# tontinton/dbeel

Measured on NVIDIA H100. Metric: compaction throughput MB/s (input bytes) at 1/2/4/8 H100 vs CPU shards, higher is better.
Workload: dtype u8

## Files before the change

dbeel_b200/csrc/kernels.cuh:

```cuda
#pragma once
#include <cuda_runtime.h>
#include <stdint.h>

#include "device_fns.cuh"

namespace dbeel {


struct RunDesc {
    const uint8_t *data;
    uint64_t data_len;
    uint64_t off_base;
    const uint4 *index;
    uint32_t n_in;
    uint32_t base;
};

struct Seg {
    uint32_t start, len;
};

enum : uint32_t {
    kFlagTruncated = 1u,
    kFlagUnsorted = 2u,
// ... 497 lines not shown
    }
    if (total) atomicAdd(&s_total, total);
    if (trunc) atomicAdd(&s_trunc, trunc);
    if (flags) atomicOr(&s_flags, flags);
    __syncthreads();
    for (uint32_t l = 0; l < p.n_levels; l++) {
        const uint32_t pairs = p.nseg[l + 1];
        uint32_t carry = 0;
        for (uint32_t j0 = 0; j0 < pairs; j0 += 1024) {
            const uint32_t j = j0 + tid;
            uint32_t tiles = 0;
            if (j < pairs) {
                const Seg a = p.seg[l][2 * j];
                const uint32_t blen = (2 * j + 1 < p.nseg[l]) ? p.seg[l][2 * j + 1].len : 0;
                p.seg[l + 1][j].start = a.start;
                p.seg[l + 1][j].len = a.len + blen;
                const uint32_t tl = (p.fin_tile && l + 1 == p.n_levels) ? p.fin_tile : (uint32_t)kMergeTile;
                tiles = (a.len + blen + tl - 1) / tl;
            }
            unsigned long long vb = 0, tb;
            uint32_t vc = tiles, tc;
            __syncthreads();
            block_excl_scan_1024(vb, vc, s_b, s_c, &tb, &tc);
            if (j < pairs) p.tile_base[l][j] = carry + vc;
            carry += tc;
        }
        if (tid == 0) p.tile_base[l][pairs] = carry;
        __syncthreads();
    }
    if (tid == 0) {
        c->total = s_total;
        c->span = p.n_groups ? p.n_total : s_total;
        c->runs_truncated = s_trunc;
        c->flags = c->flags | s_flags;
    }
}


__global__ void k_flush_prefix_init(Params p) {
    pdl_trigger();
    pdl_wait();
    if (threadIdx.x || blockIdx.x) return;
    Ctl *c = p.ctl;
    const uint8_t *ptr;
    uint32_t kl = 0;
    uint32_t L = 0;
    const RunDesc &rd = p.runs[p.flush_ref_run];
    if (rd.n_in && safe_key(rd, 0, &ptr, &kl)) {
        L = kl < kMaxPrefix ? kl : kMaxPrefix;
        for (uint32_t i = 0; i < L; i++) c->prefix[i] = __ldg(ptr + i);
    }
    c->prefix_len = L;
}

__global__ void __launch_bounds__(256) k_flush_prefix(Params p) {
    pdl_trigger();
    pdl_wait();
    Ctl *c = p.ctl;
    uint32_t g = blockIdx.x * 256u + threadIdx.x;
    uint32_t L = c->prefix_len;
    if (g < p.n_total && L) {
        const uint32_t r = find_run(p, g);
        const uint8_t *ptr;
        uint32_t kl;
        if (safe_key(p.runs[r], g - p.runs[r].base, &ptr, &kl)) {
            uint32_t m = kl < L ? kl : L, i = 0;
            while (i < m && __ldg(ptr + i) == c->prefix[i]) i++;
            L = i;
        }
    }
    for (int o = 16; o; o >>= 1) {
        uint32_t other = __shfl_xor_sync(0xFFFFFFFFu, L, o);
        L = other < L ? other : L;
    }
    if ((threadIdx.x & 31) == 0 && L < c->prefix_len) atomicMin(&c->prefix_len, L);
}

__device__ __forceinline__ bool arrival_less(const Params &p, uint32_t skip, const Rec &a, const Rec &b) {
    int und;
    int c = rec_cmp_window(a, b, &und);
    if (und) c = full_key_cmp(p, a.w, b.w, skip);
    return c < 0 || (c == 0 && a.w < b.w);
}

__global__ void __launch_bounds__(kMergeThreads) k_block_sort(Params p) {
    pdl_trigger();
    pdl_wait();
    __shared__ Rec s[kMergeTile + kMergeVT + 1];
    const Seg sg = p.seg[0][blockIdx.x];
    const uint32_t base = sg.start;
    const uint32_t n = sg.len;
    if (n == 0) return;
    const uint32_t tid = threadIdx.x;
    const uint32_t skip = p.ctl->prefix_len + kWindowBytes;
    Rec inf;
    inf.x = inf.y = inf.z = inf.w = 0xFFFFFFFFu;
    for (uint32_t i = tid; i < (uint32_t)kMergeTile; i += kMergeThreads) s[i] = i < n ? ld_rec(&p.rec_a[base + i]) : inf;
    __syncthreads();
    Rec r[kMergeVT];
#pragma unroll
    for (int i = 0; i < kMergeVT; i++) r[i] = s[tid * kMergeVT + i];
#pragma unroll
    for (int pass = 0; pass < kMergeVT; pass++) {
#pragma unroll
        for (int i = pass & 1; i + 1 < kMergeVT; i += 2) {
            if (arrival_less(p, skip, r[i + 1], r[i])) { Rec t = r[i]; r[i] = r[i + 1]; r[i + 1] = t; }
        }
    }
    __syncthreads();
#pragma unroll
    for (int i = 0; i < kMergeVT; i++) s[tid * kMergeVT + i] = r[i];
    __syncthreads();
    for (uint32_t len = kMergeVT; len < (uint32_t)kMergeTile; len <<= 1) {
        const uint32_t d0 = tid * kMergeVT;
        const uint32_t pair = d0 / (2 * len);
        const uint32_t diag = d0 - pair * 2 * len;
        const Rec *A = s + pair * 2 * len;
        const Rec *B = A + len;
        uint32_t lo = diag > len ? diag - len : 0;
        uint32_t hi = diag < len ? diag : len;
        while (lo < hi) {
            uint32_t mid = (lo + hi) >> 1;
            if (!arrival_less(p, skip, B[diag - 1 - mid], A[mid])) lo = mid + 1; else hi = mid;
        }
        uint32_t ai = lo, bi = diag - lo;
        Rec ak = A[ai < len ? ai : len - 1], bk = B[bi < len ? bi : len - 1];
#pragma unroll
        for (int i = 0; i < kMergeVT; i++) {
            bool has_a = ai < len, has_b = bi < len;
            bool take_b = has_b && (!has_a || arrival_less(p, skip, bk, ak));
            r[i] = take_b ? bk : ak;
            if (take_b) { bi++; if (bi < len) bk = B[bi]; } else { ai++; if (ai < len) ak = A[ai]; }
        }
        __syncthreads();
#pragma unroll
        for (int i = 0; i < kMergeVT; i++) s[d0 + i] = r[i];
        __syncthreads();
    }
    for (uint32_t i = tid; i < n; i += kMergeThreads) st_rec(&p.rec_a[base + i], s[i]);
}


__device__ __forceinline__ uint32_t find_pair(const uint32_t *tb, uint32_t pairs, uint32_t v, uint32_t slope) {
    uint32_t lo = 0, hi = pairs;
    while (hi - lo > 1) {
        uint32_t mid = (lo + hi) >> 1;
        if (tb[mid] + slope * mid <= v) lo = mid; else hi = mid;
    }
    return lo;
}

constexpr int kPartitionThreads = 256;

__global__ void __launch_bounds__(kPartitionThreads) k_merge_partition(Params p, uint32_t level, const Rec *src) {
    pdl_trigger();
    pdl_wait();
    const uint32_t pairs = p.nseg[level + 1];
    const uint32_t *tb = p.tile_base[level];
    const uint32_t n_bound = tb[pairs] + pairs;
    const uint32_t idx = (blockIdx.x * (uint32_t)kPartitionThreads + threadIdx.x) >> 5, lane = threadIdx.x & 31;
    if (idx >= n_bound) return;
    const uint32_t skip = p.ctl->prefix_len + kWindowBytes;
    uint32_t j = find_pair(tb, pairs, idx, 1);
    uint32_t t = idx - (tb[j] + j);
    Seg a = p.seg[level][2 * j];
    Seg b;
    b.start = 0; b.len = 0;
    if (2 * j + 1 < p.nseg[level]) b = p.seg[level][2 * j + 1];
    const bool fin = p.fin_tile && level + 1 == p.n_levels;
    uint64_t d64 = (uint64_t)t * (fin ? p.fin_tile : (uint32_t)kMergeTile);
    uint32_t n = a.len + b.len;
    uint32_t diag = d64 < n ? (uint32_t)d64 : n;
    uint32_t lo = diag > b.len ? diag - b.len : 0;
    uint32_t hi = diag < a.len ? diag : a.len;
    while (lo < hi) {
        const uint32_t range = hi - lo;
        const uint32_t step = range >= 32 ? range >> 5 : 1;
        const uint32_t mid = lo + lane * step + (step - 1);
        bool pr = false;
        if (mid < hi) {
            Rec ra = ld_rec(&src[a.start + mid]);
            Rec rb = ld_rec(&src[b.start + (diag - 1 - mid)]);
            pr = !key_less(p, skip, rb, ra);
        }
        const uint32_t cnt = __popc(__ballot_sync(0xFFFFFFFFu, pr));
        const uint32_t first_false = lo + cnt * step + (step - 1);
        lo = lo + cnt * step;
        if (cnt < 32 && first_false < hi) hi = first_false;
        else if (range < 32) hi = lo;
    }
    if (lane == 0) {
        p.part[idx] = lo;
        if (!fin) p.bnd[idx] = make_uint4(a.start + lo, b.start + (diag - lo), a.start + diag, j);
        if (t * (uint64_t)(fin ? p.fin_tile : (uint32_t)kMergeTile) < n) p.tile_bnd[tb[j] + t] = idx;
    }
    if (fin) {
        uint32_t ext = 0;
        if (diag > 0 && diag < n) {
            const uint32_t ai = lo, bi = diag - lo;
            Rec K;
            if (ai == 0) K = ld_rec(&src[b.start + bi - 1]);
            else if (bi == 0) K = ld_rec(&src[a.start + ai - 1]);
            else {
                const Rec ka = ld_rec(&src[a.start + ai - 1]), kb = ld_rec(&src[b.start + bi - 1]);
                K = key_less(p, skip, ka, kb) ? kb : ka;
            }
            const bool ea = ai + lane < a.len && key_equal(p, skip, K, ld_rec(&src[a.start + ai + lane]));
            const bool eb = bi + lane < b.len && key_equal(p, skip, K, ld_rec(&src[b.start + bi + lane]));
            const uint32_t ma = __ballot_sync(0xFFFFFFFFu, ea), mb = __ballot_sync(0xFFFFFFFFu, eb);
            uint32_t xa = (uint32_t)__ffs((int)~ma), xb = (uint32_t)__ffs((int)~mb);
            xa = xa ? xa - 1 : 32;
            xb = xb ? xb - 1 : 32;
            ext = (xa > 31 ? 31u : xa) | ((xb > 31 ? 31u : xb) << 8);
        }
        if (lane == 0) {
            p.part_ext[idx] = ext;
            p.bnd[idx] = make_uint4(a.start + lo + (ext & 0xFF), b.start + (diag - lo) + (ext >> 8), a.start + diag, j);
        }
    }
}

__global__ void __launch_bounds__(kMergeThreads, 4) k_merge(Params p, uint32_t level, const Rec *src, Rec *dst) {
    pdl_trigger();
    pdl_wait();
    __shared__ Rec s[kMergeTile + kMergeVT + 1];
    const uint32_t pairs = p.nseg[level + 1];
    const uint32_t *tb = p.tile_base[level];
    const uint32_t tile = blockIdx.x;
    if (tile >= tb[pairs]) return;
    const uint32_t tid = threadIdx.x;
    const uint32_t skip = p.ctl->prefix_len + kWindowBytes;
    uint32_t j = find_pair(tb, pairs, tile, 0);
    uint32_t t = tile - tb[j];
    Seg a = p.seg[level][2 * j];
    Seg b;
    b.start = 0; b.len = 0;
    if (2 * j + 1 < p.nseg[level]) b = p.seg[level][2 * j + 1];
    const uint32_t pidx = tb[j] + j + t;
    const uint32_t a0 = p.part[pidx], a1 = p.part[pidx + 1];
    const uint32_t total = a.len + b.len;
    const uint32_t diag0 = t * kMergeTile;
    const uint32_t diag1 = diag0 + kMergeTile < total ? diag0 + kMergeTile : total;
    const uint32_t b0 = diag0 - a0, b1 = diag1 - a1;
    const uint32_t nA = a1 - a0, nB = b1 - b0, n = nA + nB;

    for (uint32_t i = tid; i < nA; i += kMergeThreads) s[i] = ld_rec(&src[a.start + a0 + i]);
    for (uint32_t i = tid; i < nB; i += kMergeThreads) s[nA + i] = ld_rec(&src[b.start + b0 + i]);
    __syncthreads();

    uint32_t d = tid * kMergeVT;
    if (d > n) d = n;
    uint32_t lo = d > nB ? d - nB : 0;
    uint32_t hi = d < nA ? d : nA;
    while (lo < hi) {
        uint32_t mid = (lo + hi) >> 1;
        if (!key_less_smem(p, skip, &s[nA + d - 1 - mid], &s[mid])) lo = mid + 1; else hi = mid;
    }
    uint32_t ai = lo, bi = d - lo;
    Rec ak = s[ai], bk = s[nA + bi];
    Rec out[kMergeVT];
#pragma unroll
    for (int i = 0; i < kMergeVT; i++) {
        bool has_a = ai < nA, has_b = bi < nB;
        bool take_b = has_b && (!has_a || key_less(p, skip, bk, ak));
        out[i] = take_b ? bk : ak;
        if (take_b) { bi++; bk = s[nA + bi]; } else { ai++; ak = s[ai]; }
    }
    Rec *o = dst + a.start + diag0;
    __syncthreads();
#pragma unroll
    for (int i = 0; i < kMergeVT; i++)
        if (d + i < n) s[d + i] = out[i];
    __syncthreads();
    for (uint32_t i = tid; i < n; i += kMergeThreads) st_rec(&o[i], s[i]);
}


struct MergeDesc {
    uint32_t a_src, n_a, b_src, n_b, dst;
};

__device__ __forceinline__ MergeDesc merge_desc(const Params &p, uint32_t level, uint32_t tile) {
    const uint32_t pairs = p.nseg[level + 1];
    const uint32_t *tb = p.tile_base[level];
    MergeDesc d;
    d.a_src = d.n_a = d.b_src = d.n_b = d.dst = 0;
    if (tile >= tb[pairs]) return d;
    const uint32_t j = find_pair(tb, pairs, tile, 0);
    const uint32_t t = tile - tb[j];
    const Seg a = p.seg[level][2 * j];
    Seg b;
    b.start = 0; b.len = 0;
    if (2 * j + 1 < p.nseg[level]) b = p.seg[level][2 * j + 1];
    const uint32_t pidx = tb[j] + j + t;
    const uint32_t a0 = p.part[pidx], a1 = p.part[pidx + 1];
    const uint32_t total = a.len + b.len;
    const uint32_t diag0 = t * kMergeTile;
    const uint32_t diag1 = diag0 + kMergeTile < total ? diag0 + kMergeTile : total;
    d.a_src = a.start + a0;
    d.n_a = a1 - a0;
    d.b_src = b.start + (diag0 - a0);
    d.n_b = (diag1 - a1) - (diag0 - a0);
    d.dst = a.start + diag0;
    return d;
}

constexpr int kMergeBufRecs = kMergeTile + kMergeVT + 1;


__device__ __forceinline__ uint32_t smem_u32(const void *p) { return (uint32_t)__cvta_generic_to_shared(p); }
__device__ __forceinline__ void mbar_init(uint64_t *bar, uint32_t count) {
    asm volatile("mbarrier.init.shared::cta.b64 [%0], %1;" ::"r"(smem_u32(bar)), "r"(count) : "memory");
}
__device__ __forceinline__ void mbar_expect_tx(uint64_t *bar, uint32_t bytes) {
    asm volatile("mbarrier.arrive.expect_tx.shared::cta.b64 _, [%0], %1;" ::"r"(smem_u32(bar)), "r"(bytes) : "memory");
}
__device__ __forceinline__ bool mbar_try_wait(uint64_t *bar, uint32_t parity) {
    uint32_t ok;
    asm volatile("{\n .reg .pred p;\n mbarrier.try_wait.parity.shared::cta.b64 p, [%1], %2;\n selp.u32 %0, 1, 0, p;\n}"
                 : "=r"(ok) : "r"(smem_u32(bar)), "r"(parity) : "memory");
    return ok != 0;
}
__device__ __forceinline__ void tma_load_1d(void *smem_dst, const void *gmem_src, uint32_t bytes, uint64_t *bar) {
    asm volatile("cp.async.bulk.shared::cluster.global.mbarrier::complete_tx::bytes [%0], [%1], %2, [%3];" ::"r"(smem_u32(smem_dst)),
                 "l"(gmem_src), "r"(bytes), "r"(smem_u32(bar)) : "memory");
}
__device__ __forceinline__ void tma_store_1d(void *gmem_dst, const void *smem_src, uint32_t bytes) {
    asm volatile("cp.async.bulk.global.shared::cta.bulk_group [%0], [%1], %2;" ::"l"(gmem_dst), "r"(smem_u32(smem_src)), "r"(bytes) : "memory");
}

__global__ void __launch_bounds__(kMergeThreads, kMergeCtasPerSM) k_merge_tma(Params p, uint32_t level, const Rec *src, Rec *dst) {
    pdl_trigger();
    pdl_wait();
    extern __shared__ __align__(128) uint8_t s_raw[];
    Rec *bufs[2] = {reinterpret_cast<Rec *>(s_raw), reinterpret_cast<Rec *>(s_raw) + kMergeBufRecs};
    __shared__ __align__(8) uint64_t s_bar[2];
    const uint32_t tid = threadIdx.x;
    const uint32_t skip = p.ctl->prefix_len + kWindowBytes;
    const uint32_t n_tiles = p.tile_base[level][p.nseg[level + 1]];
    const uint32_t G = gridDim.x;
    uint32_t tile = blockIdx.x;
    if (tile >= n_tiles) return;
    if (tid == 0) {
        mbar_init(&s_bar[0], 1);
        mbar_init(&s_bar[1], 1);
        asm volatile("fence.mbarrier_init.release.cluster;" ::: "memory");
    }
    __syncthreads();

    auto issue = [&](const MergeDesc &d, Rec *buf, uint64_t *bar) {
        mbar_expect_tx(bar, (d.n_a + d.n_b) * 16u);
        if (d.n_a) tma_load_1d(buf, &src[d.a_src], d.n_a * 16u, bar);
        if (d.n_b) tma_load_1d(buf + d.n_a, &src[d.b_src], d.n_b * 16u, bar);
    };

    auto ld_bidx = [&](uint32_t t) -> uint32_t { return t < n_tiles ? __ldg(&p.tile_bnd[t]) : 0xFFFFFFFFu; };
    auto mk_desc = [&](uint32_t bidx) -> MergeDesc {
        MergeDesc d;
        d.a_src = d.n_a = d.b_src = d.n_b = d.dst = 0;
        if (bidx == 0xFFFFFFFFu) return d;
        const uint4 b0 = __ldg(&p.bnd[bidx]), b1 = __ldg(&p.bnd[bidx + 1]);
        d.a_src = b0.x; d.n_a = b1.x - b0.x;
        d.b_src = b0.y; d.n_b = b1.y - b0.y;
        d.dst = b0.z;
        return d;
    };
    MergeDesc cur = mk_desc(ld_bidx(tile));
    MergeDesc nxt = mk_desc(ld_bidx(tile + G));
    uint32_t bidx2 = ld_bidx(tile + 2 * G);
    if (tid == 0) issue(cur, bufs[0], &s_bar[0]);
    for (uint32_t q = 0;; q++) {
        Rec *s = bufs[q & 1];
        const bool has_next = tile + G < n_tiles;
        if (tid == 0 && has_next) {
            asm volatile("cp.async.bulk.wait_group.read 0;" ::: "memory");
            issue(nxt, bufs[(q + 1) & 1], &s_bar[(q + 1) & 1]);
        }
        const MergeDesc nn = mk_desc(bidx2);
        const uint32_t bidx3 = ld_bidx(tile + 3 * G);
        while (!mbar_try_wait(&s_bar[q & 1], (q >> 1) & 1)) {}

        const uint32_t nA = cur.n_a, nB = cur.n_b, n = nA + nB;
        uint32_t d = tid * kMergeVT;
        if (d > n) d = n;
        uint32_t lo = d > nB ? d - nB : 0;
        uint32_t hi = d < nA ? d : nA;
        while (lo < hi) {
            uint32_t mid = (lo + hi) >> 1;
            if (!key_less_smem(p, skip, &s[nA + d - 1 - mid], &s[mid])) lo = mid + 1; else hi = mid;
        }
        uint32_t ai = lo, bi = d - lo;
        Rec ak = s[ai], bk = s[nA + bi];
        Rec out[kMergeVT];
#pragma unroll
        for (int i = 0; i < kMergeVT; i++) {
            bool has_a = ai < nA, has_b = bi < nB;
            bool take_b = has_b && (!has_a || key_less(p, skip, bk, ak));
            out[i] = take_b ? bk : ak;
            if (take_b) { bi++; bk = s[nA + bi]; } else { ai++; ak = s[ai]; }
        }
        __syncthreads();
#pragma unroll
        for (int i = 0; i < kMergeVT; i++)
            if (d + i < n) s[d + i] = out[i];
        asm volatile("fence.proxy.async.shared::cta;" ::: "memory");
        __syncthreads();
        if (tid == 0) {
            tma_store_1d(dst + cur.dst, s, n * 16u);
            asm volatile("cp.async.bulk.commit_group;" ::: "memory");
        }
        if (!has_next) break;
        tile += G;
        cur = nxt;
        nxt = nn;
        bidx2 = bidx3;
    }
    if (tid == 0) asm volatile("cp.async.bulk.wait_group 0;" ::: "memory");
}


__device__ __forceinline__ void ld_ts(const uint8_t *entry, uint32_t full_size, uint64_t *lo, uint64_t *hi) {
    const uint8_t *t = entry + full_size - 16;
    *lo = ld_u64_unaligned(t);
    *hi = ld_u64_unaligned(t + 8);
}

#ifndef DBEEL_RESOLVE_MINB
#define DBEEL_RESOLVE_MINB 14
#endif
constexpr unsigned long long kScanAgg = 1, kScanPrefix = 2;

__device__ __forceinline__ unsigned long long ld_volatile_u64(const unsigned long long *q) {
    unsigned long long v;
    asm volatile("ld.volatile.global.u64 %0, [%1];" : "=l"(v) : "l"(q) : "memory");
    return v;
}
__device__ __forceinline__ void st_volatile_u64(unsigned long long *q, unsigned long long v) {
    asm volatile("st.volatile.global.u64 [%0], %1;" ::"l"(q), "l"(v) : "memory");
}

#ifndef DBEEL_RESOLVE_FUSED_MINB
#define DBEEL_RESOLVE_FUSED_MINB 12
#endif
template <bool kNarrow, bool kFused, bool kHashRec>
__global__ void __launch_bounds__(kResolveThreads, kFused ? DBEEL_RESOLVE_FUSED_MINB : DBEEL_RESOLVE_MINB) k_resolve(Params p, const Rec *m, uint4 *res) {
    pdl_trigger();
    pdl_wait();
    constexpr int NT = kResolveThreads;
    __shared__ Rec s_rec[NT + 2];
    __shared__ unsigned long long s_entry[NT];
    __shared__ uint32_t s_ks[NT], s_fs[NT];
    __shared__ unsigned long long s_tlo[NT], s_thi[NT];
    __shared__ uint8_t s_eqn[NT];
    const Ctl *c = p.ctl;
    const uint32_t tid = threadIdx.x;
    const uint32_t span = c->span;
    __shared__ uint32_t s_tile;
    if (kFused) {
        if (tid == 0) s_tile = atomicAdd(p.scan_ticket, 1u);
        __syncthreads();
    }
    const uint32_t tile_id = kFused ? s_tile : blockIdx.x;
    const uint32_t i0 = tile_id * NT;
    if (i0 >= span) return;
    const uint32_t skip = c->prefix_len + kWindowBytes;
    const uint32_t i = i0 + tid;
    uint32_t lim_lo = 0, lim_hi = c->total;
    int keep_tombstones = p.keep_tombstones;
    if (p.n_groups && i < span) {
        const uint32_t g = find_group(p, i);
        const Seg sl = p.seg[p.n_levels][g];
        lim_lo = sl.start;
        lim_hi = sl.start + sl.len;
        if (p.groups) keep_tombstones = p.groups[g].keep_tombstones;
    }

    for (uint32_t k = tid; k < NT + 2; k += NT) {
        int64_t gi = (int64_t)i0 - 1 + k;
        if (gi >= 0 && gi < (int64_t)span) s_rec[k] = ld_rec(&m[gi]);
    }
    __syncthreads();

    const bool active = i < span && i < lim_hi;
    bool eq_prev = false, eq_next = false;
// ... 1352 lines not shown
```

dbeel_b200/csrc/merge_final.cuh:

```cuda
#pragma once
#include "kernels.cuh"

namespace dbeel {

constexpr int kFinThreads = kMergeThreads;
constexpr int kFinVT = kMergeVT;
constexpr int kFinTile = kMergeTile;
constexpr int kFinNominal = kFinTile - 64;
constexpr int kFinBufRecs = kFinTile + 8;
constexpr int kFinMaxRunsSmem = 64;
#ifndef DBEEL_FIN_CTAS
#define DBEEL_FIN_CTAS 2
#endif
constexpr uint32_t kFinSmem = 2u * kFinBufRecs * 16u + 2u * kFinTile * 8u + (uint32_t)kFinTile + 16u;

struct FinDesc {
    uint32_t a_src, n_a, b_src, n_b;
    uint32_t a_end, b_end;
    uint32_t diag0;
    uint32_t nb;
};

template <bool kNarrow>
__global__ void __launch_bounds__(kFinThreads, DBEEL_FIN_CTAS) k_merge_final(Params p, uint32_t level, const Rec *src) {
    constexpr int NT = kFinThreads, VT = kFinVT;
    extern __shared__ __align__(128) uint8_t f_raw[];
    Rec *bufs[2] = {reinterpret_cast<Rec *>(f_raw), reinterpret_cast<Rec *>(f_raw) + kFinBufRecs};
    unsigned long long *s_tlo = reinterpret_cast<unsigned long long *>(f_raw + 2u * kFinBufRecs * 16u);
    unsigned long long *s_thi = s_tlo + kFinTile;
    uint8_t *s_flag = reinterpret_cast<uint8_t *>(s_thi + kFinTile);
    __shared__ __align__(8) uint64_t s_bar[2];
    __shared__ Rec s_bnd[5];
    __shared__ unsigned long long s_wb[NT / 32];
    __shared__ uint32_t s_wc[NT / 32];
    __shared__ unsigned long long s_pref_b;
    __shared__ uint32_t s_pref_c;
    __shared__ uint32_t s_first[NT / 32];
    __shared__ uint32_t s_rbase[kFinMaxRunsSmem + 1];
    __shared__ uint8_t s_rlut[256];
    __shared__ const uint4 *s_rindex[kFinMaxRunsSmem];
    __shared__ const uint8_t *s_rdata[kFinMaxRunsSmem];

    pdl_trigger();
    pdl_wait();
    const uint32_t tid = threadIdx.x, lane = tid & 31, warp = tid >> 5;
    const uint32_t skip = p.ctl->prefix_len + kWindowBytes;
    const uint32_t n_tiles = p.tile_base[level][p.nseg[level + 1]];
    const uint32_t G = gridDim.x;
    uint32_t tile = blockIdx.x;
    if (tile >= n_tiles) return;
    const bool runs_cached = p.n_runs <= (uint32_t)kFinMaxRunsSmem;
    uint32_t lut_shift = 0;
    while (((uint64_t)p.n_total >> lut_shift) > 256) lut_shift++;
    if (runs_cached) {
        for (uint32_t r = tid; r < p.n_runs; r += NT) {
            s_rbase[r] = p.runs[r].base;
            s_rindex[r] = p.runs[r].index;
            s_rdata[r] = p.runs[r].data;
        }
        if (tid == 0) s_rbase[p.n_runs] = 0xFFFFFFFFu;
        s_rlut[tid] = (uint8_t)find_run(p, (uint32_t)(((uint64_t)tid << lut_shift) < p.n_total ? (uint64_t)tid << lut_shift : p.n_total - 1));
    }
    if (tid == 0) {
        mbar_init(&s_bar[0], 1);
        mbar_init(&s_bar[1], 1);
        asm volatile("fence.mbarrier_init.release.cluster;" ::: "memory");
    }
    __syncthreads();

    auto run_of = [&](uint32_t gid) -> uint32_t {
        if (!runs_cached) return find_run(p, gid);
        uint32_t r = s_rlut[gid >> lut_shift];
        while (s_rbase[r + 1] <= gid) r++;
        return r;
    };
    auto index_ptr = [&](uint32_t gid, uint32_t r) -> const uint4 * {
        return runs_cached ? s_rindex[r] + (gid - s_rbase[r]) : p.runs[r].index + (gid - p.runs[r].base);
    };
    auto data_ptr = [&](uint32_t r) -> const uint8_t * { return runs_cached ? s_rdata[r] : p.runs[r].data; };

    auto issue = [&](const FinDesc &d, Rec *buf, uint64_t *bar) {
        const uint32_t ap = d.nb & 1u, an = (d.nb >> 1) & 1u, bp = (d.nb >> 2) & 1u, bn = (d.nb >> 3) & 1u;
        const uint32_t ca = d.n_a + ap + an, cb = d.n_b + bp + bn;
        asm volatile("fence.proxy.async.shared::cta;" ::: "memory");
        mbar_expect_tx(bar, (ca + cb) * 16u);
        if (ca) tma_load_1d(buf + 1 - ap, &src[d.a_src - ap], ca * 16u, bar);
        if (cb) tma_load_1d(buf + d.n_a + 3 - bp, &src[d.b_src - bp], cb * 16u, bar);
    };

    const Seg segA = p.seg[level][0];
    Seg segB;
    segB.start = 0; segB.len = 0;
    if (p.nseg[level] > 1) segB = p.seg[level][1];
    auto ld_bidx = [&](uint32_t t) -> uint32_t { return t < n_tiles ? __ldg(&p.tile_bnd[t]) : 0xFFFFFFFFu; };
    auto mk_desc = [&](uint32_t bidx) -> FinDesc {
        FinDesc d;
        d.a_src = d.n_a = d.b_src = d.n_b = d.a_end = d.b_end = d.diag0 = d.nb = 0;
        if (bidx == 0xFFFFFFFFu) return d;
        const uint4 b0 = __ldg(&p.bnd[bidx]), b1 = __ldg(&p.bnd[bidx + 1]);
        d.a_src = b0.x; d.n_a = b1.x - b0.x;
        d.b_src = b0.y; d.n_b = b1.y - b0.y;
        d.a_end = segA.start + segA.len;
        d.b_end = segB.start + segB.len;
        d.diag0 = b0.z;
        d.nb = (b0.x > segA.start ? 1u : 0u) | (b1.x < d.a_end ? 2u : 0u) | (b0.y > segB.start ? 4u : 0u) | (b1.y < d.b_end ? 8u : 0u);
        return d;
    };
    FinDesc cur = mk_desc(ld_bidx(tile));
    FinDesc nxt = mk_desc(ld_bidx(tile + G));
    uint32_t bidx2 = ld_bidx(tile + 2 * G);
    if (tid == 0) issue(cur, bufs[0], &s_bar[0]);
    const int keep_tombstones = p.keep_tombstones;

    for (uint32_t q = 0;; q++) {
        Rec *s = bufs[q & 1];
        uint4 *s4 = reinterpret_cast<uint4 *>(s);
        const bool has_next = tile + G < n_tiles;
        if (tid == 0 && has_next) issue(nxt, bufs[(q + 1) & 1], &s_bar[(q + 1) & 1]);
        const FinDesc nn = mk_desc(bidx2);
        const uint32_t bidx3 = ld_bidx(tile + 3 * G);
        while (!mbar_try_wait(&s_bar[q & 1], (q >> 1) & 1)) {}

        const uint32_t nA = cur.n_a, nB = cur.n_b, n = nA + nB;
        const Rec *A = s + 1, *B = s + nA + 3;
        uint32_t d = tid * VT;
        if (d > n) d = n;
        Rec me[VT + 1];
        {
            uint32_t lo = d > nB ? d - nB : 0;
            uint32_t hi = d < nA ? d : nA;
            while (lo < hi) {
                const uint32_t mid = (lo + hi) >> 1;
                if (!key_less_smem(p, skip, &B[d - 1 - mid], &A[mid])) lo = mid + 1; else hi = mid;
            }
            uint32_t ai = lo, bi = d - lo;
            Rec ak = A[ai], bk = B[bi];
#pragma unroll
            for (int i = 0; i < VT; i++) {
                const bool has_a = ai < nA, has_b = bi < nB;
                const bool take_b = has_b && (!has_a || key_less(p, skip, bk, ak));
                me[i] = take_b ? bk : ak;
                if (take_b) { bi++; bk = B[bi]; } else { ai++; ak = A[ai]; }
            }
            if (tid == 0) {
                s_bnd[0] = s[0];
                s_bnd[1] = s[nA + 1];
                s_bnd[2] = s[nA + 2];
                s_bnd[3] = s[nA + 3 + nB];
            }
            __syncthreads();
            if (d < n) s[d] = me[0];
            if (d + VT - 1 < n) s[d + VT - 1] = me[VT - 1];
#pragma unroll
            for (int i = 0; i < VT; i++)
                if (d + i == n - 1) s_bnd[4] = me[i];
        }
        __syncthreads();

        uint32_t m_act = 0, m_eqn = 0, m_eqp = 0;
        uint32_t gidv[VT];
        uint4 irec[VT];
        {
#pragma unroll
            for (int i = 0; i < VT; i++)
                if (d + i < n) m_act |= 1u << i;
            me[VT].x = me[VT].y = me[VT].z = me[VT].w = 0;
            if (d + VT < n) me[VT] = s[d + VT];
#pragma unroll
            for (int i = 0; i < VT; i++) {
                if (!(m_act & (1u << i))) continue;
                bool eqn;
                if (d + i + 1 < n) {
                    eqn = key_equal(p, skip, me[i], me[i + 1]);
                } else {
                    eqn = ((cur.nb & 2u) && key_equal(p, skip, me[i], s_bnd[1])) || ((cur.nb & 8u) && key_equal(p, skip, me[i], s_bnd[3]));
                }
                if (eqn) m_eqn |= 1u << i;
            }
            m_eqp = m_eqn << 1;
            if (m_act & 1u) {
                bool eqp;
                if (d > 0) eqp = key_equal(p, skip, s[d - 1], me[0]);
                else eqp = ((cur.nb & 1u) && key_equal(p, skip, s_bnd[0], me[0])) || ((cur.nb & 4u) && key_equal(p, skip, s_bnd[2], me[0]));
                if (eqp) m_eqp |= 1u;
            }
#pragma unroll
            for (int i = 0; i < VT; i++) {
                gidv[i] = me[i].w;
                irec[i] = make_uint4(0, 0, 0, 0);
                if (m_act & (1u << i)) {
                    const uint32_t r = run_of(gidv[i]);
                    const uint4 *q4 = index_ptr(gidv[i], r);
                    irec[i] = kNarrow ? ldg128_narrow(q4) : __ldg(q4);
                }
            }
        }
        __syncthreads();
        uint4 we[VT];
        {
            const uint32_t m_grp = m_act & (m_eqn | m_eqp);
            unsigned long long tlo[VT], thi[VT];
#pragma unroll
            for (int i = 0; i < VT; i++) {
                tlo[i] = thi[i] = 0;
                we[i] = make_uint4(0, 0, 0, 0);
                if (!(m_act & (1u << i))) continue;
                const uint32_t r = run_of(gidv[i]);
                const uint8_t *entry = data_ptr(r) + ((uint64_t)irec[i].x | ((uint64_t)irec[i].y << 32));
                const unsigned long long ea = (unsigned long long)(uintptr_t)entry;
                we[i] = make_uint4((uint32_t)ea, (uint32_t)(ea >> 32), irec[i].z, irec[i].w);
                if ((m_grp >> i) & 1u) {
                    const uint8_t *t = entry + irec[i].w - 16;
                    if (kNarrow) { tlo[i] = ld_u64_unaligned_narrow(t); thi[i] = ld_u64_unaligned_narrow(t + 8); }
                    else { tlo[i] = ld_u64_unaligned(t); thi[i] = ld_u64_unaligned(t + 8); }
                    s4[d + i] = we[i];
                    s_flag[d + i] = (uint8_t)((m_eqn >> i) & 1u);
                }
            }
#pragma unroll
            for (int i = 0; i < VT; i++) {
                if ((m_grp >> i) & 1u) { s_tlo[d + i] = tlo[i]; s_thi[d + i] = thi[i]; }
            }
        }
        __syncthreads();

        unsigned long long vb = 0;
        uint32_t vc = 0;
#pragma unroll
        for (int i = 0; i < VT; i++) {
            uint4 info = we[i];
            we[i].w = 0;
            if (!((m_act >> i) & 1u) || ((m_eqp >> i) & 1u)) continue;
            const uint32_t k = d + i;
            if ((m_eqn >> i) & 1u) {
                unsigned long long wlo = s_tlo[k], whi = s_thi[k];
                uint32_t j = k;
                bool more = true;
                while (more && j + 1 < n) {
                    j++;
                    const unsigned long long clo = s_tlo[j], chi = s_thi[j];
                    if (!ts_greater(wlo, whi, clo, chi)) { info = s4[j]; wlo = clo; whi = chi; }
                    more = s_flag[j] != 0;
                }
                if (more) {
                    const Rec last = s_bnd[4];
                    for (int side = 0; side < 2; side++) {
                        uint32_t g = side ? cur.b_src + nB : cur.a_src + nA;
                        const uint32_t end = side ? cur.b_end : cur.a_end;
                        for (; g < end; g++) {
                            const Rec nx = ld_rec(&src[g]);
                            if (!key_equal(p, skip, last, nx)) break;
                            const KeyRef ck = key_of_gid(p, nx.w);
                            uint64_t clo, chi;
                            ld_ts(ck.entry, ck.full_size, &clo, &chi);
                            if (!ts_greater(wlo, whi, clo, chi)) {
                                const unsigned long long ea = (unsigned long long)(uintptr_t)ck.entry;
                                info = make_uint4((uint32_t)ea, (uint32_t)(ea >> 32), ck.klen + 8, ck.full_size);
                                wlo = clo; whi = chi;
                            }
                        }
                    }
                }
            }
            const bool tomb = info.w == info.z + 24;
            if (keep_tombstones || !tomb) {
                we[i] = info;
                vb += info.w;
                vc += 1;
            }
        }

        unsigned long long ib = vb;
        uint32_t ic = vc;
#pragma unroll
        for (int o = 1; o < 32; o <<= 1) {
            const unsigned long long xb = __shfl_up_sync(0xFFFFFFFFu, ib, o);
            const uint32_t xc = __shfl_up_sync(0xFFFFFFFFu, ic, o);
            if (lane >= (uint32_t)o) { ib += xb; ic += xc; }
        }
        if (lane == 31) { s_wb[warp] = ib; s_wc[warp] = ic; }
        __syncthreads();
        unsigned long long tb = 0, wbefore = 0;
        uint32_t tc = 0, wcbefore = 0;
#pragma unroll
        for (int w = 0; w < NT / 32; w++) {
            if ((uint32_t)w < warp) { wbefore += s_wb[w]; wcbefore += s_wc[w]; }
            tb += s_wb[w];
            tc += s_wc[w];
        }
        unsigned long long *mine = p.scan_state + 2ull * tile;
        if (tile == 0) {
            if (tid == 0) {
                st_volatile_u64(mine, (kScanPrefix << 62) | tb);
                st_volatile_u64(mine + 1, (kScanPrefix << 32) | tc);
                s_pref_b = 0;
                s_pref_c = 0;
            }
            __syncthreads();
        } else {
            if (tid == 0) {
                st_volatile_u64(mine, (kScanAgg << 62) | tb);
                st_volatile_u64(mine + 1, (kScanAgg << 32) | tc);
            }
            unsigned long long eb = 0;
            uint32_t ec = 0;
            int base = (int)tile - 1;
            while (true) {
                const int idx = base - (int)tid;
                unsigned long long vb2 = 0, vc2 = 0, stat = kScanPrefix;
                if (idx >= 0) {
                    const unsigned long long *qs = p.scan_state + 2ull * (uint32_t)idx;
                    while (true) {
                        vc2 = ld_volatile_u64(qs + 1);
                        vb2 = ld_volatile_u64(qs);
                        if ((vc2 >> 32) != 0 && (vc2 >> 32) == (vb2 >> 62)) break;
                    }
                    stat = vc2 >> 32;
                    vb2 &= (1ull << 62) - 1;
                    vc2 &= 0xFFFFFFFFull;
                }
                const uint32_t pm = __ballot_sync(0xFFFFFFFFu, stat == kScanPrefix);
                __syncthreads();
                if (lane == 0) s_first[warp] = pm ? (warp * 32u + (uint32_t)__ffs((int)pm) - 1u) : 0xFFFFFFFFu;
                __syncthreads();
                uint32_t first = 0xFFFFFFFFu;
#pragma unroll
                for (int w = 0; w < NT / 32; w++) first = s_first[w] < first ? s_first[w] : first;
                unsigned long long cb = tid <= first ? vb2 : 0ull;
                uint32_t cc = tid <= first ? (uint32_t)vc2 : 0u;
#pragma unroll
                for (int o = 16; o; o >>= 1) {
                    cb += __shfl_xor_sync(0xFFFFFFFFu, cb, o);
                    cc += __shfl_xor_sync(0xFFFFFFFFu, cc, o);
                }
                if (lane == 0) { s_wb[warp] = cb; s_wc[warp] = cc; }
                __syncthreads();
#pragma unroll
                for (int w = 0; w < NT / 32; w++) { eb += s_wb[w]; ec += s_wc[w]; }
                if (first != 0xFFFFFFFFu) break;
                base -= NT;
            }
            if (tid == 0) {
                st_volatile_u64(mine, (kScanPrefix << 62) | (eb + tb));
                st_volatile_u64(mine + 1, (kScanPrefix << 32) | (unsigned long long)(ec + tc));
                s_pref_b = eb;
                s_pref_c = ec;
            }
            __syncthreads();
        }
        const unsigned long long pref_b = s_pref_b;
        const uint32_t pref_c = s_pref_c;
        if (tile + 1 == n_tiles && tid == 0) {
            Ctl *cw = p.ctl;
            cw->out_data_len = pref_b + tb;
            cw->out_items = pref_c + tc;
        }

        {
            unsigned long long off = pref_b + wbefore + ib - vb;
            uint32_t pos = pref_c + wcbefore + ic - vc;
            constexpr unsigned long long gt = kGatherTileBytes;
#pragma unroll
            for (int i = 0; i < VT; i++) {
                const uint32_t fs = we[i].w;
                if (!fs) continue;
                const unsigned long long file_off = off + p.out_offset_base;
                p.out_index[pos] = make_uint4((uint32_t)file_off, (uint32_t)(file_off >> 32), we[i].z, fs);
                p.src_ptr[pos] = (unsigned long long)we[i].x | ((unsigned long long)we[i].y << 32);
                for (unsigned long long bq = (off + gt - 1) / gt; bq * gt < off + fs && bq < p.tile_first_n; bq++) p.tile_first[bq] = pos;
                off += fs;
                pos++;
            }
        }
        if (!has_next) break;
        asm volatile("fence.proxy.async.shared::cta;" ::: "memory");
        __syncthreads();
        tile += G;
        cur = nxt;
        nxt = nn;
        bidx2 = bidx3;
    }
}

}
```

Before: 676,400.

## Defer decoupled lookback and emit of each tile into the next iteration

Moves the decoupled-lookback prefix resolution and index emission for a tile into the next loop iteration. It now runs after that iteration's global loads are issued, so the wait on predecessor tiles overlaps useful work. Lookback becomes a single-warp routine that reads four scan entries per lane, replacing the block-wide version with several __syncthreads. Params are passed as __grid_constant__, and optional phase-timing instrumentation is added behind a macro. The cost is reusing smem tlo/thi buffers to hold the previous tile's emit data, plus a spin-wait on a tagged shared prefix, which adds ordering risk around buffer reuse.

After: 763,100 (median of 6 runs). +12.8%, better.

```diff
diff --git a/dbeel_b200/csrc/kernels.cuh b/dbeel_b200/csrc/kernels.cuh
--- a/dbeel_b200/csrc/kernels.cuh
+++ b/dbeel_b200/csrc/kernels.cuh
@@ -673,7 +673,7 @@
 
 constexpr int kPartitionThreads = 256;
 
-__global__ void __launch_bounds__(kPartitionThreads) k_merge_partition(Params p, uint32_t level, const Rec *src) {
+__global__ void __launch_bounds__(kPartitionThreads) k_merge_partition(const __grid_constant__ Params p, uint32_t level, const Rec *src) {
     pdl_trigger();
     pdl_wait();
     const uint32_t pairs = p.nseg[level + 1];
@@ -850,7 +850,7 @@
     asm volatile("cp.async.bulk.global.shared::cta.bulk_group [%0], [%1], %2;" ::"l"(gmem_dst), "r"(smem_u32(smem_src)), "r"(bytes) : "memory");
 }
 
-__global__ void __launch_bounds__(kMergeThreads, kMergeCtasPerSM) k_merge_tma(Params p, uint32_t level, const Rec *src, Rec *dst) {
+__global__ void __launch_bounds__(kMergeThreads, kMergeCtasPerSM) k_merge_tma(const __grid_constant__ Params p, uint32_t level, const Rec *src, Rec *dst) {
     pdl_trigger();
     pdl_wait();
     extern __shared__ __align__(128) uint8_t s_raw[];
diff --git a/dbeel_b200/csrc/merge_final.cuh b/dbeel_b200/csrc/merge_final.cuh
--- a/dbeel_b200/csrc/merge_final.cuh
+++ b/dbeel_b200/csrc/merge_final.cuh
@@ -14,6 +14,29 @@
 #endif
 constexpr uint32_t kFinSmem = 2u * kFinBufRecs * 16u + 2u * kFinTile * 8u + (uint32_t)kFinTile + 16u;
 
+#ifdef DBEEL_FIN_PHASES
+constexpr int kFinPhases = 8;
+__device__ unsigned long long g_fin_phase[kFinPhases];
+__device__ unsigned int g_fin_done;
+#define FIN_PH_DECL unsigned long long ph_acc[kFinPhases] = {}; long long ph_t = clock64();
+#define FIN_PH(k) do { if (tid == 0) { const long long ph_n = clock64(); ph_acc[k] += (unsigned long long)(ph_n - ph_t); ph_t = ph_n; } } while (0)
+__device__ __forceinline__ void fin_phase_flush(const unsigned long long *acc, uint32_t n_tiles) {
+    for (int k = 0; k < kFinPhases; k++) atomicAdd(&g_fin_phase[k], acc[k]);
+    __threadfence();
+    if (atomicAdd(&g_fin_done, 1u) + 1 == (gridDim.x < n_tiles ? gridDim.x : n_tiles)) {
+        __threadfence();
+        unsigned long long v[kFinPhases], tot = 0;
+        for (int k = 0; k < kFinPhases; k++) { v[k] = atomicExch(&g_fin_phase[k], 0ull); tot += v[k]; }
+        g_fin_done = 0;
+        printf("fin_phases ctas=%u cycles=%llu tma=%llu merge=%llu index_issue=%llu index_wait=%llu lookback=%llu emit=%llu "
+               "ts_wait=%llu heads_scan=%llu\n", gridDim.x, tot, v[0], v[1], v[2], v[3], v[4], v[5], v[6], v[7]);
+    }
+}
+#else
+#define FIN_PH_DECL
+#define FIN_PH(k) do {} while (0)
+#endif
+
 struct FinDesc {
     uint32_t a_src, n_a, b_src, n_b;
     uint32_t a_end, b_end;
@@ -21,8 +44,55 @@
     uint32_t nb;
 };
 
+__device__ __forceinline__ void fin_lookback(const unsigned long long *scan_state, uint32_t t, uint32_t lane, unsigned long long &eb,
+                                             uint32_t &ec) {
+    constexpr int kPer = 4;
+    eb = 0;
+    ec = 0;
+    for (int base = (int)t - 1;; base -= 32 * kPer) {
+        unsigned long long vb[kPer], vc[kPer];
+#pragma unroll
+        for (int k = 0; k < kPer; k++) {
+            const int idx = base - (int)lane * kPer - k;
+            vb[k] = kScanPrefix << 62;
+            vc[k] = kScanPrefix << 32;
+            if (idx >= 0) {
+                vc[k] = ld_volatile_u64(scan_state + 2ull * (uint32_t)idx + 1);
+                vb[k] = ld_volatile_u64(scan_state + 2ull * (uint32_t)idx);
+            }
+        }
+        bool found = false;
+        unsigned long long sb = 0;
+        uint32_t sc = 0;
+#pragma unroll
+        for (int k = 0; k < kPer; k++) {
+            const int idx = base - (int)lane * kPer - k;
+            while ((vc[k] >> 32) == 0 || (vc[k] >> 32) != (vb[k] >> 62)) {
+                vc[k] = ld_volatile_u64(scan_state + 2ull * (uint32_t)idx + 1);
+                vb[k] = ld_volatile_u64(scan_state + 2ull * (uint32_t)idx);
+            }
+            if (!found) {
+                sb += vb[k] & ((1ull << 62) - 1);
+                sc += (uint32_t)vc[k];
+                found = (vc[k] >> 32) == kScanPrefix;
+            }
+        }
+        const uint32_t fm = __ballot_sync(0xFFFFFFFFu, found);
+        const uint32_t first = fm ? (uint32_t)__ffs((int)fm) - 1u : 32u;
+        if (lane > first) { sb = 0; sc = 0; }
+#pragma unroll
+        for (int o = 16; o; o >>= 1) {
+            sb += __shfl_xor_sync(0xFFFFFFFFu, sb, o);
+            sc += __shfl_xor_sync(0xFFFFFFFFu, sc, o);
+        }
+        eb += sb;
+        ec += sc;
+        if (fm) return;
+    }
+}
+
 template <bool kNarrow>
-__global__ void __launch_bounds__(kFinThreads, DBEEL_FIN_CTAS) k_merge_final(Params p, uint32_t level, const Rec *src) {
+__global__ void __launch_bounds__(kFinThreads, DBEEL_FIN_CTAS) k_merge_final(const __grid_constant__ Params p, uint32_t level, const Rec *src) {
     constexpr int NT = kFinThreads, VT = kFinVT;
     extern __shared__ __align__(128) uint8_t f_raw[];
     Rec *bufs[2] = {reinterpret_cast<Rec *>(f_raw), reinterpret_cast<Rec *>(f_raw) + kFinBufRecs};
@@ -33,9 +103,7 @@
     __shared__ Rec s_bnd[5];
     __shared__ unsigned long long s_wb[NT / 32];
     __shared__ uint32_t s_wc[NT / 32];
-    __shared__ unsigned long long s_pref_b;
-    __shared__ uint32_t s_pref_c;
-    __shared__ uint32_t s_first[NT / 32];
+    __shared__ unsigned long long s_pref[2];
     __shared__ uint32_t s_rbase[kFinMaxRunsSmem + 1];
     __shared__ uint8_t s_rlut[256];
     __shared__ const uint4 *s_rindex[kFinMaxRunsSmem];
@@ -64,9 +132,11 @@
     if (tid == 0) {
         mbar_init(&s_bar[0], 1);
         mbar_init(&s_bar[1], 1);
+        s_pref[0] = s_pref[1] = ~0ull;
         asm volatile("fence.mbarrier_init.release.cluster;" ::: "memory");
     }
     __syncthreads();
+    FIN_PH_DECL
 
     auto run_of = [&](uint32_t gid) -> uint32_t {
         if (!runs_cached) return find_run(p, gid);
@@ -112,7 +182,57 @@
     if (tid == 0) issue(cur, bufs[0], &s_bar[0]);
     const int keep_tombstones = p.keep_tombstones;
 
-    for (uint32_t q = 0;; q++) {
+    uint32_t prev_tile = 0, prev_d = 0, prev_act = 0, prev_pos = 0, prev_tc = 0;
+    unsigned long long prev_off = 0, prev_tb = 0;
+    volatile unsigned long long *vpref = s_pref;
+    auto finish_prev = [&](uint32_t prev_q) {
+        const unsigned long long tag = prev_q & 0xFFFFu;
+        if (warp == 0) {
+            unsigned long long eb = 0;
+            uint32_t ec = 0;
+            if (prev_tile > 0) fin_lookback(p.scan_state, prev_tile, lane, eb, ec);
+            if (lane == 0) {
+                if (prev_tile > 0) {
+                    unsigned long long *mine = p.scan_state + 2ull * prev_tile;
+                    st_volatile_u64(mine, (kScanPrefix << 62) | (eb + prev_tb));
+                    st_volatile_u64(mine + 1, (kScanPrefix << 32) | (unsigned long long)(ec + prev_tc));
+                }
+                vpref[0] = (tag << 48) | eb;
+                vpref[1] = (tag << 32) | ec;
+                if (prev_tile + 1 == n_tiles) {
+                    Ctl *cw = p.ctl;
+                    cw->out_data_len = eb + prev_tb;
+                    cw->out_items = ec + prev_tc;
+                }
+            }
+        }
+        unsigned long long pb, pc;
+        do {
+            pb = vpref[0];
+            pc = vpref[1];
+        } while ((pb >> 48) != tag || (pc >> 32) != tag);
+        FIN_PH(4);
+        unsigned long long off = (pb & ((1ull << 48) - 1)) + prev_off;
+        uint32_t pos = (uint32_t)pc + prev_pos;
+        constexpr unsigned long long gt = kGatherTileBytes;
+#pragma unroll
+        for (int i = 0; i < VT; i++) {
+            if (!((prev_act >> i) & 1u)) continue;
+            const unsigned long long sz = s_thi[prev_d + i];
+            const uint32_t fs = (uint32_t)(sz >> 32);
+            if (!fs) continue;
+            const unsigned long long file_off = off + p.out_offset_base;
+            p.out_index[pos] = make_uint4((uint32_t)file_off, (uint32_t)(file_off >> 32), (uint32_t)sz, fs);
+            p.src_ptr[pos] = s_tlo[prev_d + i];
+            for (unsigned long long bq = (off + gt - 1) / gt; bq * gt < off + fs && bq < p.tile_first_n; bq++) p.tile_first[bq] = pos;
+            off += fs;
+            pos++;
+        }
+        FIN_PH(5);
+    };
+
+    uint32_t q = 0;
+    for (;; q++) {
         Rec *s = bufs[q & 1];
         uint4 *s4 = reinterpret_cast<uint4 *>(s);
         const bool has_next = tile + G < n_tiles;
@@ -120,6 +240,7 @@
         const FinDesc nn = mk_desc(bidx2);
         const uint32_t bidx3 = ld_bidx(tile + 3 * G);
         while (!mbar_try_wait(&s_bar[q & 1], (q >> 1) & 1)) {}
+        FIN_PH(0);
 
         const uint32_t nA = cur.n_a, nB = cur.n_b, n = nA + nB;
         const Rec *A = s + 1, *B = s + nA + 3;
@@ -156,6 +277,7 @@
                 if (d + i == n - 1) s_bnd[4] = me[i];
         }
         __syncthreads();
+        FIN_PH(1);
 
         uint32_t m_act = 0, m_eqn = 0, m_eqp = 0;
         uint32_t gidv[VT];
@@ -196,42 +318,44 @@
             }
         }
         __syncthreads();
-        uint4 we[VT];
+        FIN_PH(2);
         {
             const uint32_t m_grp = m_act & (m_eqn | m_eqp);
             unsigned long long tlo[VT], thi[VT];
 #pragma unroll
             for (int i = 0; i < VT; i++) {
                 tlo[i] = thi[i] = 0;
-                we[i] = make_uint4(0, 0, 0, 0);
                 if (!(m_act & (1u << i))) continue;
                 const uint32_t r = run_of(gidv[i]);
                 const uint8_t *entry = data_ptr(r) + ((uint64_t)irec[i].x | ((uint64_t)irec[i].y << 32));
                 const unsigned long long ea = (unsigned long long)(uintptr_t)entry;
-                we[i] = make_uint4((uint32_t)ea, (uint32_t)(ea >> 32), irec[i].z, irec[i].w);
+                s4[d + i] = make_uint4((uint32_t)ea, (uint32_t)(ea >> 32), irec[i].z, irec[i].w);
                 if ((m_grp >> i) & 1u) {
                     const uint8_t *t = entry + irec[i].w - 16;
                     if (kNarrow) { tlo[i] = ld_u64_unaligned_narrow(t); thi[i] = ld_u64_unaligned_narrow(t + 8); }
                     else { tlo[i] = ld_u64_unaligned(t); thi[i] = ld_u64_unaligned(t + 8); }
-                    s4[d + i] = we[i];
                     s_flag[d + i] = (uint8_t)((m_eqn >> i) & 1u);
                 }
             }
+            FIN_PH(3);
+            if (q > 0) finish_prev(q - 1);
 #pragma unroll
             for (int i = 0; i < VT; i++) {
                 if ((m_grp >> i) & 1u) { s_tlo[d + i] = tlo[i]; s_thi[d + i] = thi[i]; }
             }
         }
         __syncthreads();
+        FIN_PH(6);
 
         unsigned long long vb = 0;
         uint32_t vc = 0;
+        uint4 we[VT];
 #pragma unroll
         for (int i = 0; i < VT; i++) {
-            uint4 info = we[i];
-            we[i].w = 0;
+            we[i] = make_uint4(0, 0, 0, 0);
             if (!((m_act >> i) & 1u) || ((m_eqp >> i) & 1u)) continue;
             const uint32_t k = d + i;
+            uint4 info = s4[k];
             if ((m_eqn >> i) & 1u) {
                 unsigned long long wlo = s_tlo[k], whi = s_thi[k];
                 uint32_t j = k;
@@ -288,98 +412,42 @@
             tb += s_wb[w];
             tc += s_wc[w];
         }
-        unsigned long long *mine = p.scan_state + 2ull * tile;
-        if (tile == 0) {
-            if (tid == 0) {
-                st_volatile_u64(mine, (kScanPrefix << 62) | tb);
-                st_volatile_u64(mine + 1, (kScanPrefix << 32) | tc);
-                s_pref_b = 0;
-                s_pref_c = 0;
-            }
-            __syncthreads();
-        } else {
-            if (tid == 0) {
-                st_volatile_u64(mine, (kScanAgg << 62) | tb);
-                st_volatile_u64(mine + 1, (kScanAgg << 32) | tc);
-            }
-            unsigned long long eb = 0;
-            uint32_t ec = 0;
-            int base = (int)tile - 1;
-            while (true) {
-                const int idx = base - (int)tid;
-                unsigned long long vb2 = 0, vc2 = 0, stat = kScanPrefix;
-                if (idx >= 0) {
-                    const unsigned long long *qs = p.scan_state + 2ull * (uint32_t)idx;
-                    while (true) {
-                        vc2 = ld_volatile_u64(qs + 1);
-                        vb2 = ld_volatile_u64(qs);
-                        if ((vc2 >> 32) != 0 && (vc2 >> 32) == (vb2 >> 62)) break;
-                    }
-                    stat = vc2 >> 32;
-                    vb2 &= (1ull << 62) - 1;
-                    vc2 &= 0xFFFFFFFFull;
-                }
-                const uint32_t pm = __ballot_sync(0xFFFFFFFFu, stat == kScanPrefix);
-                __syncthreads();
-                if (lane == 0) s_first[warp] = pm ? (warp * 32u + (uint32_t)__ffs((int)pm) - 1u) : 0xFFFFFFFFu;
-                __syncthreads();
-                uint32_t first = 0xFFFFFFFFu;
-#pragma unroll
-                for (int w = 0; w < NT / 32; w++) first = s_first[w] < first ? s_first[w] : first;
-                unsigned long long cb = tid <= first ? vb2 : 0ull;
-                uint32_t cc = tid <= first ? (uint32_t)vc2 : 0u;
-#pragma unroll
-                for (int o = 16; o; o >>= 1) {
-                    cb += __shfl_xor_sync(0xFFFFFFFFu, cb, o);
-                    cc += __shfl_xor_sync(0xFFFFFFFFu, cc, o);
-                }
-                if (lane == 0) { s_wb[warp] = cb; s_wc[warp] = cc; }
-                __syncthreads();
-#pragma unroll
-                for (int w = 0; w < NT / 32; w++) { eb += s_wb[w]; ec += s_wc[w]; }
-                if (first != 0xFFFFFFFFu) break;
-                base -= NT;
-            }
-            if (tid == 0) {
-                st_volatile_u64(mine, (kScanPrefix << 62) | (eb + tb));
-                st_volatile_u64(mine + 1, (kScanPrefix << 32) | (unsigned long long)(ec + tc));
-                s_pref_b = eb;
-                s_pref_c = ec;
-            }
-            __syncthreads();
-        }
-        const unsigned long long pref_b = s_pref_b;
-        const uint32_t pref_c = s_pref_c;
-        if (tile + 1 == n_tiles && tid == 0) {
-            Ctl *cw = p.ctl;
-            cw->out_data_len = pref_b + tb;
-            cw->out_items = pref_c + tc;
-        }
-
-        {
-            unsigned long long off = pref_b + wbefore + ib - vb;
-            uint32_t pos = pref_c + wcbefore + ic - vc;
-            constexpr unsigned long long gt = kGatherTileBytes;
-#pragma unroll
-            for (int i = 0; i < VT; i++) {
-                const uint32_t fs = we[i].w;
-                if (!fs) continue;
-                const unsigned long long file_off = off + p.out_offset_base;
-                p.out_index[pos] = make_uint4((uint32_t)file_off, (uint32_t)(file_off >> 32), we[i].z, fs);
-                p.src_ptr[pos] = (unsigned long long)we[i].x | ((unsigned long long)we[i].y << 32);
-                for (unsigned long long bq = (off + gt - 1) / gt; bq * gt < off + fs && bq < p.tile_first_n; bq++) p.tile_first[bq] = pos;
-                off += fs;
-                pos++;
-            }
-        }
-        if (!has_next) break;
+        if (tid == 0) {
+            const unsigned long long st = tile == 0 ? kScanPrefix : kScanAgg;
+            unsigned long long *mine = p.scan_state + 2ull * tile;
+            st_volatile_u64(mine, (st << 62) | tb);
+            st_volatile_u64(mine + 1, (st << 32) | tc);
+        }
+#pragma unroll
+        for (int i = 0; i < VT; i++) {
+            if ((m_act >> i) & 1u) {
+                s_tlo[d + i] = (unsigned long long)we[i].x | ((unsigned long long)we[i].y << 32);
+                s_thi[d + i] = (unsigned long long)we[i].z | ((unsigned long long)we[i].w << 32);
+            }
+        }
+        prev_tile = tile;
+        prev_d = d;
+        prev_act = m_act;
+        prev_off = wbefore + ib - vb;
+        prev_pos = wcbefore + ic - vc;
+        prev_tb = tb;
+        prev_tc = tc;
+        if (!has_next) {
+            FIN_PH(7);
+            break;
+        }
         asm volatile("fence.proxy.async.shared::cta;" ::: "memory");
         __syncthreads();
+        FIN_PH(7);
         tile += G;
         cur = nxt;
         nxt = nn;
         bidx2 = bidx3;
     }
+    finish_prev(q);
+#ifdef DBEEL_FIN_PHASES
+    if (tid == 0) fin_phase_flush(ph_acc, n_tiles);
+#endif
 }
 
 }
```
